# vislearn/HINT

Measured on AMD Instinct MI355X. Metric: train_samples_per_sec, higher is better.
Workload: dtype f32; 1 GPU; power_hint_8: d=6, 8 recursive coupling blocks, c_internal=[140, 70, 35, 17], batch 4096 per GPU; global_batch=4096, parallelism=dp1, hip_graph=True, steps_per_graph=1, input=batch resident in the captured step's input buffer (no per-step copy), rccl_world_size=1, backend=none (one process), gradient_allreduce=none (one process: clamp + Adam ride in the weight gradients' final reduction)

## Files before the change

hint_amd/csrc/hint_wl.hpp:

```cpp
#pragma once
#include "hint_rows.hpp"

namespace hint {

__device__ __forceinline__ f32x4 fma4(const f32x4 w, float s, const f32x4 a) {
    return f32x4{fmaf(w.x, s, a.x), fmaf(w.y, s, a.y), fmaf(w.z, s, a.z), fmaf(w.w, s, a.w)};
}
__device__ __forceinline__ float dot4(const f32x4 w, const f32x4 v, float a) {
    return fmaf(w.w, v.w, fmaf(w.z, v.z, fmaf(w.y, v.y, fmaf(w.x, v.x, a))));
}
__device__ __forceinline__ f32x4 relu4(const f32x4 v) { return f32x4{fmaxf(v.x, 0.f), fmaxf(v.y, 0.f), fmaxf(v.z, 0.f), fmaxf(v.w, 0.f)}; }
__device__ __forceinline__ f32x4 relu4m(const f32x4 v) {
    return f32x4{__builtin_amdgcn_fmed3f(v.x, 0.f, 3.0e38f), __builtin_amdgcn_fmed3f(v.y, 0.f, 3.0e38f),
                 __builtin_amdgcn_fmed3f(v.z, 0.f, 3.0e38f), __builtin_amdgcn_fmed3f(v.w, 0.f, 3.0e38f)};
}
__device__ __forceinline__ float kq_sum(float v) {
    const unsigned u = (unsigned)__float_as_int(v);
    const auto h = __builtin_amdgcn_permlane32_swap(u, u, false, false);
    const float a = __int_as_float((int)h[0]) + __int_as_float((int)h[1]);
    const unsigned ua = (unsigned)__float_as_int(a);
    const auto q = __builtin_amdgcn_permlane16_swap(ua, ua, false, false);
    return __int_as_float((int)q[0]) + __int_as_float((int)q[1]);
}

template <bool TRANS, typename WP>
__device__ __forceinline__ void wl_perm(float* dst, const float* src, int ld, WP w, int d, int lane) {
    const int m = lane & 15, kq = lane >> 4;
    float av[4], bv[4];
#pragma unroll
    for (int t = 0; t < 4; ++t) {
        const int k = 4 * t + kq;
        const int kc = k < d ? k : 0, mc = m < d ? m : 0;
        av[t] = TRANS ? w[mc * d + kc] : w[kc * d + mc];
        bv[t] = src[m * ld + kc];
    }
    f32x4 acc = zero4();
#pragma unroll
    for (int t = 0; t < 4; ++t) {
        if (4 * t < d) {
            const bool ok = 4 * t + kq < d;
            acc = mfma4((ok && m < d) ? av[t] : 0.f, ok ? bv[t] : 0.f, acc);
        }
    }
#pragma unroll
    for (int i = 0; i < 4; ++i)
        if (4 * kq + i < d) dst[m * ld + 4 * kq + i] = acc[i];
}

__device__ __forceinline__ void wl_store_share(float* __restrict__ dst, const float* tile, int ld, int d, float inv_d, int nvalid,
                                               int wave, int nw, int lane) {
    const int per = (ROWS * d + nw - 1) / nw;
    const int i = wave * per + lane;
    if (lane < per && i < nvalid) { const int r = fdiv(i, inv_d); dst[i] = tile[r * ld + (i - r * d)]; }
}

typedef unsigned wl_u32x4 __attribute__((ext_vector_type(4)));
__device__ __forceinline__ f32x4 wl_as_f32x4(wl_u32x4 v) { return __builtin_bit_cast(f32x4, v); }
__device__ __forceinline__ void wl_mask_by_bits(f32x4& v, int bits) {
    const float e[4] = {v.x, v.y, v.z, v.w};
    float o[4];
#pragma unroll
    for (int i = 0; i < 4; ++i) o[i] = __int_as_float(__float_as_int(e[i]) & __builtin_amdgcn_sbfe(bits, i, 1));
    v = f32x4{o[0], o[1], o[2], o[3]};
}

__device__ __forceinline__ f32x4 wl_layer1(const LDS_AS f32x4* q, const float (&vin)[4]) {
    const f32x4 qb = q[16], q0 = q[0], q1 = q[4], q2 = q[8], q3 = q[12];
    return fma4(q3, vin[3], fma4(q2, vin[2], fma4(q1, vin[1], fma4(q0, vin[0], qb))));
}

struct WlCtx {
    const GLOBAL_AS float* pk;
    const GLOBAL_AS float* pk_next;
    const GLOBAL_AS uint8_t* bits[2];
    const GLOBAL_AS uint8_t* bits_next[2];
    const LDS_AS int32_t* lrecs;
    const LDS_AS float* par;
    LDS_AS float* slab;
    const LDS_AS float* xs[2];
    const LDS_AS float* gst[2];
    LDS_AS float* scratch;
    GLOBAL_AS float* a2[2];
    GLOBAL_AS uint8_t* bits_out[2];
    GLOBAL_AS float* tw;
    int xld, gld, WT, slab_h;
    int sid, sid0;
    bool train, first_tile;
};

template <int KIND, int NR>
__device__ __forceinline__ void wl_load(f32x4 (&dst)[NEL], const GLOBAL_AS float* pk, const GLOBAL_AS uint8_t* const (&bits)[2],
                                        const RowU& r, int kb, const LaneOff& lo) {
    const __amdgpu_buffer_rsrc_t rw = __builtin_amdgcn_make_buffer_rsrc((void*)pk, 0, -1, 0x00020000);
#pragma unroll
    for (int j = 0; j < NTT; ++j) {
        const int jj = j < r.ntt ? j : r.ntt - 1;
        dst[j] = wl_as_f32x4(__builtin_amdgcn_raw_buffer_load_b128(rw, (int)lo.w, (r.base1 + jj * r.n1 + kb) * 1024, 0));
    }
// ... 194 lines not shown
    RecV nrec;
};
template <int KIND, int NR>
__device__ __forceinline__ void wl_rows(const WlCtx& c, f32x4 (&ring)[RING][NEL], WlCarry& cy, int r0, int r1, int rnext,
                                        bool other_block, int lane) {
    if (r0 >= r1) return;
    LaneOff lo;
    lo.w = (unsigned)lane * 16u; lo.b = (unsigned)(lane >> 4) * 16u; lo.l = (unsigned)lane;
    if (cy.held != r0) cy.nrec = wl_rec_fetch(c.lrecs, r0, lane);
    RowU cr = wl_rec_decode(cy.nrec);
    if (cy.primed != r0) wl_load<KIND, NR>(ring[0], c.pk, c.bits, cr, 0, lo);
    const int rlast = rnext >= 0 ? rnext : r1 - 1;
    cy.nrec = wl_rec_fetch(c.lrecs, r0 + 1 < r1 ? r0 + 1 : rlast, lane);
    f32x4 part[NR];
#pragma unroll
    for (int h = 0; h < NR; ++h) part[h] = zero4();
    for (int t = r0; t < r1; ++t) {
        const RowU nr = wl_rec_decode(cy.nrec);
        cy.nrec = wl_rec_fetch(c.lrecs, t + 2 < r1 ? t + 2 : rlast, lane);
        const bool hand = t + 1 == r1 && other_block;
#ifdef HINT_STAMPS
        const_cast<WlCtx&>(c).sid = 256 + ((c.sid0 >> 3) & 3) * 64 + (t - r0 < 2 ? t - r0 : 1) * 32;
#endif
        const GLOBAL_AS float* pkn = hand ? c.pk_next : c.pk;
        const GLOBAL_AS uint8_t* const bitsn[2] = {hand ? c.bits_next[0] : c.bits[0], hand ? c.bits_next[1] : c.bits[1]};
        wl_row<KIND, NR>(c, cr, nr, pkn, bitsn, ring, part, lo, lane);
        cr = nr;
    }
    cy.primed = rnext;
    cy.held = rlast;
}

template <int PR>
__device__ __forceinline__ void wl_par_issue(f32x4 (&pf)[PR], const GLOBAL_AS float* packed, const WlArgs& w, int tid, int nthreads) {
#pragma unroll
    for (int q = 0; q < PR; ++q) {
        int i = tid + q * nthreads;
        i = i < w.par_f4 ? i : w.par_f4 - 1;
        const int f = 4 * i;
        pf[q] = *(const GLOBAL_AS f32x4*)(packed + (f < w.par_bias ? f : f - w.par_bias + w.bias_src));
    }
}
__device__ __forceinline__ void wl_par_dma(const GLOBAL_AS float* packed, const WlArgs& w, const LDS_AS float* dst, int wave, int nw, int lane) {
    const int nchunk = (w.par_f4 + 63) >> 6;
    const unsigned base = (unsigned)(unsigned long long)dst;
    for (int c = wave; c < nchunk; c += nw) {
        int i = c * 64 + lane;
        i = i < w.par_f4 ? i : w.par_f4 - 1;
        const int f = 4 * i;
        const GLOBAL_AS float* src = packed + (f < w.par_bias ? f : f - w.par_bias + w.bias_src);
        const unsigned ldsb = (unsigned)rfl((int)(base + (unsigned)c * 1024u));
        unsigned keep;
        asm volatile("s_mov_b32 %0, m0\n\ts_mov_b32 m0, %2\n\ts_nop 0\n\tglobal_load_lds_dwordx4 %1, off\n\ts_mov_b32 m0, %0"
                     : "=&s"(keep) : "v"(src), "s"(ldsb) : "memory");
    }
}
__device__ __forceinline__ void wl_par_dma_wait() { asm volatile("s_waitcnt vmcnt(0)" ::: "memory"); }
template <int PR>
__device__ __forceinline__ void wl_par_commit(const f32x4 (&pf)[PR], float* dst, const WlArgs& w, int tid, int nthreads) {
#pragma unroll
    for (int q = 0; q < PR; ++q) {
        const int i = tid + q * nthreads;
        if (i < w.par_f4) ((f32x4*)dst)[i] = pf[q];
    }

}

}
```

hint_amd/csrc/hint_wl_bwd.hip:

```cpp
#include "hint_wl.hpp"

using namespace hint;

struct WlLevel { float x[WL_LV], s[WL_LV]; };
__device__ __forceinline__ void wl_level_issue(WlLevel& p, const float* __restrict__ xsrc, const float* __restrict__ ssrc,
                                               int d, int row0, int nvalid, int lane) {
    const size_t base = (size_t)row0 * d;
#pragma unroll
    for (int k = 0; k < WL_LV; ++k) {
        const int i = lane + 64 * k;
        const int ic = i < nvalid ? i : 0;
        p.x[k] = xsrc[base + ic];
        p.s[k] = ssrc[base + ic];
    }
}
__device__ __forceinline__ void wl_level_commit(const WlLevel& p, float* xs, float* sb, int ld, int d, int nvalid, int lane) {
    const float inv = frcp(d);
#pragma unroll
    for (int k = 0; k < WL_LV; ++k) {
        const int i = lane + 64 * k;
        if (i < ROWS * d) {
            const int r = fdiv(i, inv), j = i - r * d;
            xs[r * ld + j] = i < nvalid ? p.x[k] : 0.f;
            sb[r * ld + j] = i < nvalid ? p.s[k] : 0.f;
        }
    }
}

template <int NR, bool CH>
__global__ __launch_bounds__(64 * MAX_NW) __attribute__((amdgpu_waves_per_eu(2, 2))) void hint_wl_bwd_kernel(
    KArgs a, WlArgs w, ChainBlock one, const ChainBlock* __restrict__ chain, int n_chain,
    const float* __restrict__ x, const float* __restrict__ g_z, const float* __restrict__ g_J,
    float* __restrict__ g_x, float gz_scale, float gJ_const) {
    extern __shared__ __attribute__((aligned(16))) float lds[];
    const int tid = threadIdx.x, nthreads = blockDim.x;
    const int lane = tid & 63;
    const int wave = rfl(tid >> 6);
    const float inv_d = frcp(a.d);
    const Tables T = make_tables(a, lds);
    float* par = lds + w.off_par;
    float* slabs = lds + w.off_slab;
    float* ptab = lds + w.off_perm;
    float* gj = lds + w.off_misc;
    float* priv = lds + w.off_priv + wave * w.priv_stride;
    const int tl = ROWS * a.xld;
#define XSP(H) (priv + (H) * w.priv_tile)
#define SBP(H) (priv + (H) * w.priv_tile + tl)
#define G0P(H) (priv + (H) * w.priv_tile + 2 * tl)
#define GSTP(H) (priv + (H) * w.priv_tile + 4 * tl)
    float* scratch = priv + NR * w.priv_tile;
    const int par_floats = (4 * w.par_f4 + 255) & ~255;
    const int ntiles = (a.B + ROWS - 1) / ROWS;
    const int ngroups = (ntiles + NR - 1) / NR;
    const int pdd = a.d * a.d;
    const size_t lvl = (size_t)a.B * a.d;
    STAMP_DECL()
    copy_meta(a, lds, tid, nthreads);
    LDS_AS int32_t* lrecs = (LDS_AS int32_t*)(lds + w.off_recs);
    wl_stage_recs(lrecs, (const char*)a.recs + (size_t)a.total_rows * sizeof(RowRec), a.total_rows, tid, nthreads);
    if (a.perm_lds > 0) {
        for (int i = tid; i < n_chain * pdd; i += nthreads) {
            const int cbi = fdiv(i, frcp(pdd));
            const float* pp = CH ? chain[cbi].perm : one.perm;
            ptab[i] = pp != nullptr ? ((const GLOBAL_AS float*)pp)[i - cbi * pdd] : 0.f;
        }
    }
#define HINT_CB(I) chain_block<CH ? 1 : 2>(chain, one, I)
    int tr0 = 0, tr1 = 0, tgi = 0;
    bool tabs_ready = false;
#define LEVEL_SRC(TAPE, TOP, LV) ((LV) == 0 ? ((TOP) ? (TAPE) + (size_t)(a.n_levels - 1) * lvl : x) : (TAPE) + (size_t)((LV) - 1) * lvl)
#define BITS_A2(BLK, R0) ((const GLOBAL_AS uint8_t*)((BLK).actA1 + a.bits_off) + a.bits_stride + (size_t)((R0) >> 4) * (a.WT >> 4) * 64)

    for (int tg = blockIdx.x; tg < ngroups; tg += gridDim.x) {
        int row0[NR], nvalid[NR], rowt[NR];
#pragma unroll
        for (int h = 0; h < NR; ++h) {
            row0[h] = (tg * NR + h) * ROWS;
            const int rows = a.B - row0[h];
            nvalid[h] = (rows < 0 ? 0 : rows < ROWS ? rows : ROWS) * a.d;
            rowt[h] = row0[h] < ntiles * ROWS ? row0[h] : row0[0];
        }
        int gcur = 0;
#define GS(H) (G0P(H) + gcur)
#define GO(H) (G0P(H) + (tl - gcur))
#pragma unroll
        for (int h = 0; h < NR; ++h)
            for (int i = lane; i < ROWS * a.d; i += 64) {
                const int r = fdiv(i, inv_d);
                GS(h)[r * a.xld + (i - r * a.d)] = i < nvalid[h] ? g_z[(size_t)row0[h] * a.d + i] * gz_scale : 0.f;
            }
        if (tid < ROWS * NR) {
            const int h = tid >> 4, r = tid & 15;
            gj[tid] = ((tg * NR + h) * ROWS + r < a.B) ? (g_J != nullptr ? g_J[(tg * NR + h) * ROWS + r] : gJ_const) : 0.f;
        }
        {
            const GBlock lb = HINT_CB(n_chain - 1);
            const float* tape = (const float*)lb.tape;
            const bool top = lb.perm != nullptr || n_chain > 1;
            WlLevel lp[NR];
#pragma unroll
            for (int h = 0; h < NR; ++h)
                wl_level_issue(lp[h], LEVEL_SRC(tape, top, a.n_levels - 1), tape + (size_t)(2 * a.n_levels - 1) * lvl, a.d, rowt[h], nvalid[h], lane);
            f32x4 pf[NR == 2 ? WL_PAR_REGS2 : WL_PAR_REGS];
            wl_par_issue(pf, lb.packed, w, tid, nthreads);
#pragma unroll
            for (int h = 0; h < NR; ++h) wl_level_commit(lp[h], XSP(h), SBP(h), a.xld, a.d, nvalid[h], lane);
            wl_par_commit(pf, par, w, tid, nthreads);
        }
        __syncthreads();
        if (!tabs_ready) {
            const int b = lane <= a.n_groups ? lane : 0;
            const LDS_AS int32_t* gp = (const LDS_AS int32_t*)(T.groups + (b < a.n_groups ? b : 0));
            const int row_begin = gp[3], rngb = gp[6];
            tr0 = row_begin + T.rng[rngb + wave];
            tr1 = row_begin + T.rng[rngb + wave + 1];
            tgi = gp[7] | (T.rng[a.lop_cnt + b] << 8);
            tabs_ready = true;
        }
        int phase = 0;
        WlCarry primed; primed.primed = -1; primed.held = -1;
        f32x4 ring[RING][NEL];

        for (int cb = n_chain - 1; cb >= 0; --cb) {
            const int wi = n_chain - 1 - cb;
            const bool has_next = cb > 0;
            const GBlock blk = HINT_CB(cb);
            const GBlock nblk = HINT_CB(has_next ? cb - 1 : cb);
            const float* perm = (const float*)blk.perm;
            const float* tape = (const float*)blk.tape;
            const bool top = perm != nullptr || cb > 0;
            float* wsGST = (float*)blk.wsGST;
            const int tsel = wi & (a.nw - 1);
            constexpr bool PAR_DMA = NR == 2;
            f32x4 pf[PAR_DMA ? 1 : WL_PAR_REGS];
            if constexpr (PAR_DMA) { if (has_next) wl_par_dma(nblk.packed, w, (const LDS_AS float*)(par + ((wi + 1) & 1) * par_floats), wave, a.nw, lane); }
            else wl_par_issue(pf, nblk.packed, w, tid, nthreads);

            WlCtx c;
            c.pk = blk.packed; c.pk_next = nblk.packed;
#pragma unroll
            for (int h = 0; h < 2; ++h) {
                const int hh = h < NR ? h : 0;
                c.bits[h] = BITS_A2(blk, rowt[hh]); c.bits_next[h] = BITS_A2(nblk, rowt[hh]);
                c.xs[h] = (const LDS_AS float*)XSP(hh); c.gst[h] = (const LDS_AS float*)GSTP(hh);
                c.a2[h] = nullptr; c.bits_out[h] = nullptr;
            }
            c.lrecs = lrecs;
            c.par = (const LDS_AS float*)(par + (wi & 1) * par_floats);
            c.scratch = (LDS_AS float*)scratch;
            c.tw = blk.wsSlab + a.thin_slab_off + (size_t)blockIdx.x * a.tw_floats;
            c.xld = a.xld; c.gld = a.gld; c.WT = a.WT; c.slab_h = w.slab_floats; c.train = true; c.first_tile = tg == (int)blockIdx.x;

            for (int gi = a.n_groups; gi >= 0; --gi) {
                const int slot = gi > 0 ? gi - 1 : a.n_groups;
                const bool tail_only = gi == 0;
                const int ginfo = wl_lane_get(tgi, slot);
                struct { int level; } g;
                g.level = ginfo & 0xff;
                const int lop0 = slot * a.d;
                const float* slab_prev = slabs + ((phase + 1) & 1) * NR * w.slab_floats;
                const int sid = (wi * (a.n_groups + 1) + (a.n_groups - gi)) * 8;
                (void)sid;
                STAMP(sid + 0)
                const int nact = ginfo >> 8;
                for (int idx = lane; idx < ROWS * nact; idx += 64) {
                    const int row = idx & 15, kk = idx >> 4;
// ... 24 lines not shown
#pragma unroll
                                for (int u = 0; u < 4; ++u) gb[h] += u < sl_n ? v[u] : 0.f;
                                if (more) for (int sl = 4; sl < sl_n; ++sl) gb[h] += sp[sl * 64];
                            }
                        }
#pragma unroll
                        for (int h = 0; h < NR; ++h) {
                            if (colb == col) gval[h] = gb[h];
                            else GS(h)[row * a.xld + colb] = gb[h];
                        }
                    }
                    if (!tail_only && cp_ls >= 0) {
#pragma unroll
                        for (int h = 0; h < NR; ++h) {
                            const float s = SBP(h)[row * a.xld + col];
                            const float aa = a.alpha * atanf(s);
                            const float ea = expf(aa);
                            const float l = XSP(h)[row * a.xld + col];
                            const float ga = gval[h] * ea * l + gj[h * ROWS + row];
                            const float gsv = ga * a.alpha * __builtin_amdgcn_rcpf(1.f + s * s);
                            GSTP(h)[row * a.gld + cp_ls] = gsv;
                            GSTP(h)[row * a.gld + cp_lt] = gval[h];
                            if (wave == tsel && row0[h] < ntiles * ROWS) {
                                float* go = wsGST + (size_t)(row0[h] + row) * a.ST;
                                go[cp_gs] = gsv;
                                go[cp_gt] = gval[h];
                            }
                            gval[h] *= ea;
                        }
                    }
#pragma unroll
                    for (int h = 0; h < NR; ++h) GS(h)[row * a.xld + col] = gval[h];
                }
                c.sid0 = sid; c.sid = 256;
                STAMP(sid + 1)
                if (tail_only) break;

                WlLevel lp[NR];
                bool lp_pending = false;
                {
                    const bool block_switch = slot == 0;
                    int nlevel = a.n_levels - 1;
                    if (!block_switch) nlevel = wl_lane_get(tgi, slot - 1) & 0xff;
                    if (block_switch ? cb > 0 : nlevel != g.level) {
                        const float* ntape = block_switch ? (const float*)nblk.tape : tape;
                        const bool ntop = block_switch ? (nblk.perm != nullptr || cb > 1) : top;
#pragma unroll
                        for (int h = 0; h < NR; ++h)
                            wl_level_issue(lp[h], LEVEL_SRC(ntape, ntop, nlevel), ntape + (size_t)(a.n_levels + nlevel) * lvl, a.d, rowt[h], nvalid[h], lane);
                        lp_pending = true;
                    }
                }
                c.slab = (LDS_AS float*)(slabs + (phase & 1) * NR * w.slab_floats);
                ++phase;
                {
                    int rnext = -1;
                    const bool wrap = slot == 0;
                    if (!wrap || has_next) {
                        const int gn = wrap ? a.n_groups - 1 : slot - 1;
                        const int n0 = wl_lane_get(tr0, gn), n1 = wl_lane_get(tr1, gn);
                        if (n0 < n1) rnext = n0;
                    }
                    if (wave >= 4) __builtin_amdgcn_s_setprio(1);
                    wl_rows<K_BWD, NR>(c, ring, primed, wl_lane_get(tr0, slot), wl_lane_get(tr1, slot), rnext, wrap, lane);
                    __builtin_amdgcn_s_setprio(0);
                }
                STAMP(sid + 2)
                if (gi == a.n_groups) {
                    if constexpr (PAR_DMA) wl_par_dma_wait();
                    else wl_par_commit(pf, par + ((wi + 1) & 1) * par_floats, w, tid, nthreads);
                }
                if (lp_pending) {
#pragma unroll
                    for (int h = 0; h < NR; ++h) wl_level_commit(lp[h], XSP(h), SBP(h), a.xld, a.d, nvalid[h], lane);
                }
                STAMP(sid + 3)
                lds_barrier();
                STAMP(sid + 4)
            }
            if (blk.g_add != nullptr) {
#pragma unroll
                for (int h = 0; h < NR; ++h)
                    for (int i = lane; i < nvalid[h]; i += 64) {
                        const int r = fdiv(i, inv_d);
                        GS(h)[r * a.xld + (i - r * a.d)] += blk.g_add[(size_t)row0[h] * a.d + i];
                    }
            }
            if (perm != nullptr) {
#pragma unroll
                for (int h = 0; h < NR; ++h) {
                    if (a.perm_lds > 0) wl_perm<true>(GO(h), GS(h), a.xld, (const LDS_AS float*)(ptab + cb * pdd), a.d, lane);
                    else wl_perm<true>(GO(h), GS(h), a.xld, (const GLOBAL_AS float*)perm, a.d, lane);
                }
                gcur = tl - gcur;
            }
        }
        if (wave == 0) {
#pragma unroll
            for (int h = 0; h < NR; ++h)
                for (int i = lane; i < nvalid[h]; i += 64) { const int r = fdiv(i, inv_d); g_x[(size_t)row0[h] * a.d + i] = GS(h)[r * a.xld + (i - r * a.d)]; }
        }
        __syncthreads();
#undef GS
#undef GO
    }
    STAMP_FLUSH(a.stamps)
#undef HINT_CB
#undef LEVEL_SRC
#undef BITS_A2
#undef XSP
#undef SBP
#undef G0P
#undef GSTP
}

namespace hint {

hipError_t launch_wl_bwd(const KArgs& a, const WlArgs& w, int lds_bytes, int grid, const ChainBlock& one,
                         const ChainBlock* chain, int n_chain, const float* x, const float* g_z, const float* g_J,
                         float* g_x, float gz_scale, float gJ_const, hipStream_t stream) {
#define HINT_LAUNCH(NRV, CHV)                                                                                        \
    hipLaunchKernelGGL((hint_wl_bwd_kernel<NRV, CHV>), dim3(grid), dim3(64 * a.nw), lds_bytes, stream, a, w, one, chain, n_chain, x, \
                       g_z, g_J, g_x, gz_scale, gJ_const)
// ... 18 lines not shown
```

hint_amd/csrc/hint_wl_fwd.hip:

```cpp
#include "hint_wl.hpp"

using namespace hint;

template <bool REV, int NR, bool CH>
__global__ __launch_bounds__(64 * MAX_NW) __attribute__((amdgpu_waves_per_eu(2, 2))) void hint_wl_apply_kernel(
    KArgs a, WlArgs w, ChainBlock one, const ChainBlock* __restrict__ chain, int n_chain,
    const float* __restrict__ x, float* __restrict__ z, float* __restrict__ J, const float* __restrict__ J_in,
    float* __restrict__ loss_acc, float noise, const unsigned long long* __restrict__ rng_state,
    float* __restrict__ x_noisy) {
    extern __shared__ __attribute__((aligned(16))) float lds[];
    const int tid = threadIdx.x, nthreads = blockDim.x;
    const int lane = tid & 63, m = lane & 15, kq = lane >> 4;
    const int wave = rfl(tid >> 6);
    const float inv_d = frcp(a.d);
    const Tables T = make_tables(a, lds);
    float* par = lds + w.off_par;
    float* slabs = lds + w.off_slab;
    float* ptab = lds + w.off_perm;
    float* priv = lds + w.off_priv + wave * w.priv_stride;
    const int par_floats = (4 * w.par_f4 + 255) & ~255;
    const int ntiles = (a.B + ROWS - 1) / ROWS;
    const int ngroups = (ntiles + NR - 1) / NR;
    const int pdd = a.d * a.d;
    const size_t lvl = (size_t)a.B * a.d;
    STAMP_DECL()
    copy_meta(a, lds, tid, nthreads);
    LDS_AS int32_t* lrecs = (LDS_AS int32_t*)(lds + w.off_recs);
    wl_stage_recs(lrecs, a.recs, a.total_rows, tid, nthreads);
    if (a.perm_lds > 0) {
        for (int i = tid; i < n_chain * pdd; i += nthreads) {
            const int cbi = fdiv(i, frcp(pdd));
            const float* pp = CH ? chain[cbi].perm : one.perm;
            ptab[i] = pp != nullptr ? ((const GLOBAL_AS float*)pp)[i - cbi * pdd] : 0.f;
        }
    }
#define HINT_CB(I) chain_block<CH ? 1 : 2>(chain, one, I)
    int tr0 = 0, tr1 = 0, tgi = 0;
    bool tabs_ready = false;

    for (int tg = blockIdx.x; tg < ngroups; tg += gridDim.x) {
        int row0[NR], nvalid[NR];
#pragma unroll
        for (int h = 0; h < NR; ++h) {
            row0[h] = (tg * NR + h) * ROWS;
            const int rows = a.B - row0[h];
            nvalid[h] = (rows < 0 ? 0 : rows < ROWS ? rows : ROWS) * a.d;
        }
        int xcur = 0;
        const int xflip = ROWS * a.xld;
#define XS(H) (priv + (H) * w.priv_tile + xcur)
#define XO(H) (priv + (H) * w.priv_tile + (xflip - xcur))
#pragma unroll
        for (int h = 0; h < NR; ++h)
            for (int i = lane; i < ROWS * a.d; i += 64) {
                const int r = fdiv(i, inv_d);
                XS(h)[r * a.xld + (i - r * a.d)] = i < nvalid[h] ? x[(size_t)row0[h] * a.d + i] : 0.f;
            }
        if (!REV && rng_state != nullptr) {
            const unsigned long long seed = rng_state[0], step = rng_state[1];
#pragma unroll
            for (int h = 0; h < NR; ++h) {
                for (int q = lane; 4 * q < nvalid[h]; q += 64) {
                    float nz[4];
                    philox_normal4(seed, step, (unsigned)(((size_t)row0[h] * a.d) / 4 + (size_t)q), nz);
#pragma unroll
                    for (int e = 0; e < 4; ++e) {
                        const int i = 4 * q + e;
                        if (i < nvalid[h]) { const int r = fdiv(i, inv_d); XS(h)[r * a.xld + (i - r * a.d)] += noise * nz[e]; }
                    }
                }
                if (x_noisy != nullptr && wave == 0)
                    for (int i = lane; i < nvalid[h]; i += 64) { const int r = fdiv(i, inv_d); x_noisy[(size_t)row0[h] * a.d + i] = XS(h)[r * a.xld + (i - r * a.d)]; }
            }
        }
        {
            const GBlock b0 = HINT_CB(REV ? n_chain - 1 : 0);
            f32x4 pf[NR == 2 ? WL_PAR_REGS2 : WL_PAR_REGS];
            wl_par_issue(pf, b0.packed, w, tid, nthreads);
            wl_par_commit(pf, par, w, tid, nthreads);
        }
        __syncthreads();
        if (!tabs_ready) {
            const int e = lane < a.n_groups ? lane : 0;
            const LDS_AS int32_t* gp = (const LDS_AS int32_t*)(T.groups + (REV ? a.n_groups - 1 - e : e));
            const int row_begin = gp[3], rngb = gp[6];
            tr0 = row_begin + T.rng[rngb + wave];
            tr1 = row_begin + T.rng[rngb + wave + 1];
            tgi = gp[4] | (gp[5] << 16) | (gp[7] << 24) | (gp[8] << 30);
            tabs_ready = true;
        }
        float jpart[NR];
#pragma unroll
        for (int h = 0; h < NR; ++h) jpart[h] = 0.f;
        int phase = 0;
        WlCarry primed; primed.primed = -1; primed.held = -1;
        f32x4 ring[RING][NEL];

        for (int cb = 0; cb < n_chain; ++cb) {
            const int bi = REV ? n_chain - 1 - cb : cb;
            const bool has_next = cb + 1 < n_chain;
            const GBlock blk = HINT_CB(bi);
            const GBlock nblk = HINT_CB(has_next ? (REV ? bi - 1 : bi + 1) : bi);
            const float* perm = (const float*)blk.perm;
            float* tape = (float*)blk.tape;
            const bool train = !REV && blk.actA1 != nullptr;
            const int tsel = cb & (a.nw - 1);
            if (!REV && perm != nullptr) {
#pragma unroll
                for (int h = 0; h < NR; ++h) {
                    if (a.perm_lds > 0) wl_perm<false>(XO(h), XS(h), a.xld, (const LDS_AS float*)(ptab + bi * pdd), a.d, lane);
                    else wl_perm<false>(XO(h), XS(h), a.xld, (const GLOBAL_AS float*)perm, a.d, lane);
                }
                xcur = xflip - xcur;
            }
            if (!REV && tape != nullptr && (perm != nullptr || cb > 0)) {
#pragma unroll
                for (int h = 0; h < NR; ++h)
                    wl_store_share(tape + (size_t)(a.n_levels - 1) * lvl + (size_t)row0[h] * a.d, XS(h), a.xld, a.d, inv_d, nvalid[h], wave, a.nw, lane);
            }
            f32x4 pf[NR == 2 ? WL_PAR_REGS2 : WL_PAR_REGS];
            wl_par_issue(pf, nblk.packed, w, tid, nthreads);

            WlCtx c;
            c.pk = blk.packed; c.pk_next = nblk.packed;
            c.lrecs = lrecs;
            c.par = (const LDS_AS float*)(par + (cb & 1) * par_floats);
            c.scratch = nullptr; c.tw = nullptr;
#pragma unroll
            for (int h = 0; h < 2; ++h) {
                const int hh = h < NR ? h : 0;
                c.bits[h] = nullptr; c.bits_next[h] = nullptr; c.gst[h] = nullptr;
                const bool tile_ok = train && h < NR && row0[hh] < ntiles * ROWS;
                c.a2[h] = tile_ok ? blk.actA1 + a.a2_off + (size_t)row0[hh] * a.WT : nullptr;
                c.bits_out[h] = tile_ok ? (GLOBAL_AS uint8_t*)(blk.actA1 + a.bits_off) + a.bits_stride + (size_t)(row0[hh] >> 4) * (a.WT >> 4) * 64 : nullptr;
            }
            c.xld = a.xld; c.gld = 0; c.WT = a.WT; c.slab_h = w.slab_floats; c.train = train; c.first_tile = false;

            for (int gi = 0; gi < a.n_groups; ++gi) {
                const int ginfo = wl_lane_get(tgi, gi);
                struct { int ent_begin, ent_cnt, level, level_last; } g;
                g.ent_begin = ginfo & 0xffff; g.ent_cnt = (ginfo >> 16) & 0xff; g.level = (ginfo >> 24) & 0x3f; g.level_last = (ginfo >> 30) & 1;
                float* slab = slabs + (phase & 1) * NR * w.slab_floats;
                ++phase;
#pragma unroll
                for (int h = 0; h < 2; ++h) c.xs[h] = (const LDS_AS float*)XS(h < NR ? h : 0);
                c.slab = (LDS_AS float*)slab;
                const int sid = (cb * a.n_groups + gi) * 8;
                (void)sid;
                c.sid0 = sid; c.sid = 256;
                STAMP(sid + 0)
                {
                    int rnext = -1;
                    const bool wrap = gi + 1 == a.n_groups;
                    if (!wrap || has_next) {
                        const int en = wrap ? 0 : gi + 1;
                        const int n0 = wl_lane_get(tr0, en), n1 = wl_lane_get(tr1, en);
                        if (n0 < n1) rnext = n0;
// ... 27 lines not shown
#pragma unroll
                        for (int u = 0; u < 4; ++u) { s += u < sl_ns ? vs[u] : 0.f; t += u < sl_nt ? vt[u] : 0.f; }
                        if (more) {
                            for (int sl = 4; sl < sl_ns; ++sl) s += sp[sl * 64];
                            for (int sl = 4; sl < sl_nt; ++sl) t += tp[sl * 64];
                        }
                        const float aa = a.alpha * atanf(s);
                        if (act && train && tape != nullptr && wave == tsel && row0[h] + m < a.B)
                            tape[(size_t)(a.n_levels + g.level) * lvl + (size_t)(row0[h] + m) * a.d + xcol] = s;
                        float xn;
                        if (!REV) { xn = expf(aa) * xold[h] + t; jpart[h] += act ? aa : 0.f; }
                        else      { xn = (xold[h] - t) * __builtin_amdgcn_rcpf(expf(aa)); jpart[h] -= act ? aa : 0.f; }
                        if (act) XS(h)[m * a.xld + xcol] = xn;
                    }
                    if (ps + 1 < npass) {
                        const int en = 4 * (ps + 1) + kq;
                        ent = *(const LDS_AS i32x4*)(T.ents + g.ent_begin + (en < g.ent_cnt ? en : 0));
#pragma unroll
                        for (int h = 0; h < NR; ++h) xold[h] = XS(h)[m * a.xld + (ent.x & 0xffff)];
                    }
                }
                STAMP(sid + 4)
                if (gi == 0) {
                    wl_par_commit(pf, par + ((cb + 1) & 1) * par_floats, w, tid, nthreads);
                    if (a.n_groups == 1) lds_barrier();
                }
                if (!REV && tape != nullptr && g.level_last && g.level < a.n_levels - 1) {
#pragma unroll
                    for (int h = 0; h < NR; ++h)
                        wl_store_share(tape + (size_t)g.level * lvl + (size_t)row0[h] * a.d, XS(h), a.xld, a.d, inv_d, nvalid[h], wave, a.nw, lane);
                }
                STAMP(sid + 5)
            }
            if (REV && perm != nullptr) {
#pragma unroll
                for (int h = 0; h < NR; ++h) {
                    if (a.perm_lds > 0) wl_perm<true>(XO(h), XS(h), a.xld, (const LDS_AS float*)(ptab + bi * pdd), a.d, lane);
                    else wl_perm<true>(XO(h), XS(h), a.xld, (const GLOBAL_AS float*)perm, a.d, lane);
                }
                xcur = xflip - xcur;
            }
        }
        float zz = 0.f, js = 0.f;
#pragma unroll
        for (int h = 0; h < NR; ++h) {
            const bool rok = row0[h] + m < a.B;
            const float jrow = kq_sum(jpart[h]) + ((J_in != nullptr && rok) ? J_in[row0[h] + m] : 0.f);
            if (wave == 0) {
                for (int i = lane; i < nvalid[h]; i += 64) {
                    const int r = fdiv(i, inv_d);
                    const float v = XS(h)[r * a.xld + (i - r * a.d)];
                    z[(size_t)row0[h] * a.d + i] = v;
                    zz += v * v;
                }
                if (kq == 0 && rok) { J[row0[h] + m] = jrow; js += jrow; }
            }
        }
        if (wave == 0 && loss_acc != nullptr) {
            for (int o = 32; o > 0; o >>= 1) { zz += __shfl_xor(zz, o, 64); js += __shfl_xor(js, o, 64); }
            if (lane == 0) {
                float* slot = loss_acc + 2 * (blockIdx.x & 63);
                atomicAdd(slot, 0.5f * zz);
                atomicAdd(slot + 1, js);
            }
        }
        __syncthreads();
#undef XS
#undef XO
    }
    STAMP_FLUSH(a.stamps)
#undef HINT_CB
}

namespace hint {

hipError_t launch_wl_apply(bool rev, const KArgs& a, const WlArgs& w, int lds_bytes, int grid, const ChainBlock& one,
                           const ChainBlock* chain, int n_chain, const float* x, float* z, float* J, const float* J_in,
                           float* loss_acc, float noise, const unsigned long long* rng_state, float* x_noisy,
// ... 29 lines not shown
```

Before: 14.46 million samples/s.

## Pin kernel args in SGPRs, load next-block pointers lazily, rematerialize lane ids

Copies the kernel arguments into locals and pins them in scalar registers through inline-asm moves. The next chain block's pointers are now read from the constant-address-space chain array only when they are needed, and the per-tile bit-offset deltas are precomputed. Lane and thread indices are passed as separately rematerialized values so the compiler does not keep extra VGPRs live across the long loops. The goal is to cut register pressure and spills in the fused forward and backward kernels, at the cost of asm barriers that can constrain the scheduler.

After: 14.62 million samples/s, median of 6. 1.01x the previous value.

```diff
diff --git a/hint_amd/csrc/hint_wl.hpp b/hint_amd/csrc/hint_wl.hpp
--- a/hint_amd/csrc/hint_wl.hpp
+++ b/hint_amd/csrc/hint_wl.hpp
@@ -23,9 +23,29 @@
     return __int_as_float((int)q[0]) + __int_as_float((int)q[1]);
 }
 
+#if defined(__HIP_DEVICE_COMPILE__)
+#define WL_DEV_ASM(...) __VA_ARGS__
+#else
+#define WL_DEV_ASM(...)
+#endif
+template <typename T>
+__device__ __forceinline__ void wl_own(T& v) {
+    static_assert(sizeof(T) == 4 || sizeof(T) == 8, "one register or a pair");
+    T o = v;
+    if constexpr (sizeof(T) == 4) { WL_DEV_ASM(asm volatile("s_mov_b32 %0, %1" : "=s"(o) : "s"(v))); }
+    else { WL_DEV_ASM(asm volatile("s_mov_b64 %0, %1" : "=s"(o) : "s"(v))); }
+    v = o;
+}
+template <typename T>
+__device__ __forceinline__ T wl_here(T v) { WL_DEV_ASM(asm volatile("" : "+s"(v))); return v; }
+
+__device__ __forceinline__ int wl_fresh(int& lane_o) { WL_DEV_ASM(asm volatile("" : "+v"(lane_o))); return lane_o; }
+
 template <bool TRANS, typename WP>
-__device__ __forceinline__ void wl_perm(float* dst, const float* src, int ld, WP w, int d, int lane) {
+__device__ __forceinline__ void wl_perm(float* dst, const float* src, int ld, WP w, int d, int lane, int lane_f) {
     const int m = lane & 15, kq = lane >> 4;
+    const int mf = lane_f & 15, kqf = lane_f >> 4;
+    const int df = wl_here(d);
     float av[4], bv[4];
 #pragma unroll
     for (int t = 0; t < 4; ++t) {
@@ -37,21 +57,21 @@
     f32x4 acc = zero4();
 #pragma unroll
     for (int t = 0; t < 4; ++t) {
-        if (4 * t < d) {
-            const bool ok = 4 * t + kq < d;
-            acc = mfma4((ok && m < d) ? av[t] : 0.f, ok ? bv[t] : 0.f, acc);
+        if (4 * t < df) {
+            const bool ok = kqf + 4 * t < df;
+            acc = mfma4((ok && mf < df) ? av[t] : 0.f, ok ? bv[t] : 0.f, acc);
         }
     }
 #pragma unroll
     for (int i = 0; i < 4; ++i)
-        if (4 * kq + i < d) dst[m * ld + 4 * kq + i] = acc[i];
-}
-
-__device__ __forceinline__ void wl_store_share(float* __restrict__ dst, const float* tile, int ld, int d, float inv_d, int nvalid,
-                                               int wave, int nw, int lane) {
+        if (4 * kqf + i < df) dst[m * ld + 4 * kq + i] = acc[i];
+}
+
+__device__ __forceinline__ void wl_store_share(GLOBAL_AS float* __restrict__ dst, const float* tile, int ld, int d, float inv_d, int nvalid,
+                                               int wave, int nw, int lane, int lane_f) {
     const int per = (ROWS * d + nw - 1) / nw;
     const int i = wave * per + lane;
-    if (lane < per && i < nvalid) { const int r = fdiv(i, inv_d); dst[i] = tile[r * ld + (i - r * d)]; }
+    if (lane_f < per && lane_f < nvalid - wave * per) { const int r = fdiv(i, inv_d); dst[i] = tile[r * ld + (i - r * d)]; }
 }
 
 typedef unsigned wl_u32x4 __attribute__((ext_vector_type(4)));
@@ -69,11 +89,33 @@
     return fma4(q3, vin[3], fma4(q2, vin[2], fma4(q1, vin[1], fma4(q0, vin[0], qb))));
 }
 
+typedef const __attribute__((address_space(4))) ChainBlock* WlChain;
+struct WlBlk {
+    const GLOBAL_AS float* packed;
+    const GLOBAL_AS float* perm;
+    GLOBAL_AS float* tape;
+    GLOBAL_AS float* actA1;
+    GLOBAL_AS float* wsGST;
+    GLOBAL_AS float* wsSlab;
+    const GLOBAL_AS float* g_add;
+};
+#define WL_BLK_FIELD(F) ((GLOBAL_AS float*)(CH ? chain[i].F : one.F))
+template <bool CH>
+__device__ __forceinline__ WlBlk wl_block(WlChain chain, const ChainBlock& one, int i) {
+    WlBlk b;
+    b.packed = WL_BLK_FIELD(packed); b.perm = WL_BLK_FIELD(perm); b.tape = WL_BLK_FIELD(tape); b.actA1 = WL_BLK_FIELD(actA1);
+    b.wsGST = WL_BLK_FIELD(wsGST); b.wsSlab = WL_BLK_FIELD(wsSlab); b.g_add = WL_BLK_FIELD(g_add);
+    WL_DEV_ASM(asm("" : "+s"(b.packed)); asm("" : "+s"(b.perm)); asm("" : "+s"(b.tape)); asm("" : "+s"(b.actA1));
+               asm("" : "+s"(b.wsGST)); asm("" : "+s"(b.wsSlab)); asm("" : "+s"(b.g_add)));
+    return b;
+}
+#undef WL_BLK_FIELD
+
 struct WlCtx {
     const GLOBAL_AS float* pk;
-    const GLOBAL_AS float* pk_next;
+    WlChain next;
     const GLOBAL_AS uint8_t* bits[2];
-    const GLOBAL_AS uint8_t* bits_next[2];
+    long long bits_delta[2];
     const LDS_AS int32_t* lrecs;
     const LDS_AS float* par;
     LDS_AS float* slab;
@@ -314,8 +356,17 @@
 #ifdef HINT_STAMPS
         const_cast<WlCtx&>(c).sid = 256 + ((c.sid0 >> 3) & 3) * 64 + (t - r0 < 2 ? t - r0 : 1) * 32;
 #endif
-        const GLOBAL_AS float* pkn = hand ? c.pk_next : c.pk;
-        const GLOBAL_AS uint8_t* const bitsn[2] = {hand ? c.bits_next[0] : c.bits[0], hand ? c.bits_next[1] : c.bits[1]};
+        const GLOBAL_AS float* pkn = c.pk;
+        const GLOBAL_AS uint8_t* bitsn[2] = {c.bits[0], c.bits[1]};
+        if (hand && c.next != nullptr) {
+            const WlChain nx = wl_here(c.next);
+            pkn = (const GLOBAL_AS float*)nx->packed;
+            if (KIND == K_BWD) {
+                const GLOBAL_AS uint8_t* an = (const GLOBAL_AS uint8_t*)nx->actA1;
+#pragma unroll
+                for (int h = 0; h < 2; ++h) bitsn[h] = an + c.bits_delta[h < NR ? h : 0];
+            }
+        }
         wl_row<KIND, NR>(c, cr, nr, pkn, bitsn, ring, part, lo, lane);
         cr = nr;
     }
@@ -349,13 +400,13 @@
 }
 __device__ __forceinline__ void wl_par_dma_wait() { asm volatile("s_waitcnt vmcnt(0)" ::: "memory"); }
 template <int PR>
-__device__ __forceinline__ void wl_par_commit(const f32x4 (&pf)[PR], float* dst, const WlArgs& w, int tid, int nthreads) {
+__device__ __forceinline__ void wl_par_commit(const f32x4 (&pf)[PR], float* dst, const WlArgs& w, int tid, int tid_f, int nthreads) {
 #pragma unroll
     for (int q = 0; q < PR; ++q) {
         const int i = tid + q * nthreads;
-        if (i < w.par_f4) ((f32x4*)dst)[i] = pf[q];
-    }
-
-}
-
-}
+        if (tid_f + q * nthreads < w.par_f4) ((f32x4*)dst)[i] = pf[q];
+    }
+
+}
+
+}
diff --git a/hint_amd/csrc/hint_wl_bwd.hip b/hint_amd/csrc/hint_wl_bwd.hip
--- a/hint_amd/csrc/hint_wl_bwd.hip
+++ b/hint_amd/csrc/hint_wl_bwd.hip
@@ -3,7 +3,7 @@
 using namespace hint;
 
 struct WlLevel { float x[WL_LV], s[WL_LV]; };
-__device__ __forceinline__ void wl_level_issue(WlLevel& p, const float* __restrict__ xsrc, const float* __restrict__ ssrc,
+__device__ __forceinline__ void wl_level_issue(WlLevel& p, const GLOBAL_AS float* __restrict__ xsrc, const GLOBAL_AS float* __restrict__ ssrc,
                                                int d, int row0, int nvalid, int lane) {
     const size_t base = (size_t)row0 * d;
 #pragma unroll
@@ -14,28 +14,42 @@
         p.s[k] = ssrc[base + ic];
     }
 }
-__device__ __forceinline__ void wl_level_commit(const WlLevel& p, float* xs, float* sb, int ld, int d, int nvalid, int lane) {
+__device__ __forceinline__ void wl_level_commit(const WlLevel& p, float* xs, float* sb, int ld, int d, int nvalid, int lane, int lane_f) {
     const float inv = frcp(d);
 #pragma unroll
     for (int k = 0; k < WL_LV; ++k) {
         const int i = lane + 64 * k;
-        if (i < ROWS * d) {
+        const int i_f = lane_f + 64 * k;
+        if (i_f < ROWS * d) {
             const int r = fdiv(i, inv), j = i - r * d;
-            xs[r * ld + j] = i < nvalid ? p.x[k] : 0.f;
-            sb[r * ld + j] = i < nvalid ? p.s[k] : 0.f;
+            const bool ok = i_f < nvalid;
+            xs[r * ld + j] = ok ? p.x[k] : 0.f;
+            sb[r * ld + j] = ok ? p.s[k] : 0.f;
         }
     }
 }
 
 template <int NR, bool CH>
 __global__ __launch_bounds__(64 * MAX_NW) __attribute__((amdgpu_waves_per_eu(2, 2))) void hint_wl_bwd_kernel(
-    KArgs a, WlArgs w, ChainBlock one, const ChainBlock* __restrict__ chain, int n_chain,
+    KArgs a_, WlArgs w_, ChainBlock one, const ChainBlock* __restrict__ chain, int n_chain,
     const float* __restrict__ x, const float* __restrict__ g_z, const float* __restrict__ g_J,
     float* __restrict__ g_x, float gz_scale, float gJ_const) {
     extern __shared__ __attribute__((aligned(16))) float lds[];
+    KArgs a = a_;
+    WlArgs w = w_;
+    wl_own(a.d); wl_own(a.xld); wl_own(a.gld); wl_own(a.B); wl_own(a.n_levels); wl_own(a.n_groups); wl_own(a.nw); wl_own(a.alpha);
+    wl_own(a.ST); wl_own(a.WT); wl_own(a.bits_off); wl_own(a.bits_stride); wl_own(a.thin_slab_off); wl_own(a.tw_floats); wl_own(a.perm_lds);
+    WlChain chc = (WlChain)(unsigned long long)chain;
+    const GLOBAL_AS float* xg = (const GLOBAL_AS float*)x;
+    const GLOBAL_AS float* gzg = (const GLOBAL_AS float*)g_z;
+    const GLOBAL_AS float* gJg = (const GLOBAL_AS float*)g_J;
+    GLOBAL_AS float* gxg = (GLOBAL_AS float*)g_x;
+    wl_own(chc); wl_own(n_chain); wl_own(xg); wl_own(gzg); wl_own(gJg); wl_own(gxg); wl_own(gz_scale); wl_own(gJ_const);
+    wl_own(w.slab_floats); wl_own(w.priv_tile); wl_own(w.par_f4); wl_own(w.par_bias); wl_own(w.bias_src);
     const int tid = threadIdx.x, nthreads = blockDim.x;
     const int lane = tid & 63;
     const int wave = rfl(tid >> 6);
+    int lane_o = lane, tid_o = tid;
     const float inv_d = frcp(a.d);
     const Tables T = make_tables(a, lds);
     float* par = lds + w.off_par;
@@ -65,11 +79,10 @@
             ptab[i] = pp != nullptr ? ((const GLOBAL_AS float*)pp)[i - cbi * pdd] : 0.f;
         }
     }
-#define HINT_CB(I) chain_block<CH ? 1 : 2>(chain, one, I)
+#define HINT_CB(I) wl_block<CH>(chc, one, I)
     int tr0 = 0, tr1 = 0, tgi = 0;
     bool tabs_ready = false;
-#define LEVEL_SRC(TAPE, TOP, LV) ((LV) == 0 ? ((TOP) ? (TAPE) + (size_t)(a.n_levels - 1) * lvl : x) : (TAPE) + (size_t)((LV) - 1) * lvl)
-#define BITS_A2(BLK, R0) ((const GLOBAL_AS uint8_t*)((BLK).actA1 + a.bits_off) + a.bits_stride + (size_t)((R0) >> 4) * (a.WT >> 4) * 64)
+#define LEVEL_SRC(TAPE, TOP, LV) ((LV) == 0 ? ((TOP) ? (TAPE) + (size_t)(a.n_levels - 1) * lvl : xg) : (TAPE) + (size_t)((LV) - 1) * lvl)
 
     for (int tg = blockIdx.x; tg < ngroups; tg += gridDim.x) {
         int row0[NR], nvalid[NR], rowt[NR];
@@ -80,6 +93,12 @@
             nvalid[h] = (rows < 0 ? 0 : rows < ROWS ? rows : ROWS) * a.d;
             rowt[h] = row0[h] < ntiles * ROWS ? row0[h] : row0[0];
         }
+        long long bits_delta[NR];
+#pragma unroll
+        for (int h = 0; h < NR; ++h) {
+            bits_delta[h] = (long long)a.bits_off * 4 + a.bits_stride + (long long)(rowt[h] >> 4) * (a.WT >> 4) * 64;
+            wl_own(bits_delta[h]);
+        }
         int gcur = 0;
 #define GS(H) (G0P(H) + gcur)
 #define GO(H) (G0P(H) + (tl - gcur))
@@ -87,15 +106,15 @@
         for (int h = 0; h < NR; ++h)
             for (int i = lane; i < ROWS * a.d; i += 64) {
                 const int r = fdiv(i, inv_d);
-                GS(h)[r * a.xld + (i - r * a.d)] = i < nvalid[h] ? g_z[(size_t)row0[h] * a.d + i] * gz_scale : 0.f;
+                GS(h)[r * a.xld + (i - r * a.d)] = i < nvalid[h] ? gzg[(size_t)row0[h] * a.d + i] * gz_scale : 0.f;
             }
         if (tid < ROWS * NR) {
             const int h = tid >> 4, r = tid & 15;
-            gj[tid] = ((tg * NR + h) * ROWS + r < a.B) ? (g_J != nullptr ? g_J[(tg * NR + h) * ROWS + r] : gJ_const) : 0.f;
+            gj[tid] = ((tg * NR + h) * ROWS + r < a.B) ? (gJg != nullptr ? gJg[(tg * NR + h) * ROWS + r] : gJ_const) : 0.f;
         }
         {
-            const GBlock lb = HINT_CB(n_chain - 1);
-            const float* tape = (const float*)lb.tape;
+            const WlBlk lb = HINT_CB(n_chain - 1);
+            const GLOBAL_AS float* tape = lb.tape;
             const bool top = lb.perm != nullptr || n_chain > 1;
             WlLevel lp[NR];
 #pragma unroll
@@ -104,8 +123,8 @@
             f32x4 pf[NR == 2 ? WL_PAR_REGS2 : WL_PAR_REGS];
             wl_par_issue(pf, lb.packed, w, tid, nthreads);
 #pragma unroll
-            for (int h = 0; h < NR; ++h) wl_level_commit(lp[h], XSP(h), SBP(h), a.xld, a.d, nvalid[h], lane);
-            wl_par_commit(pf, par, w, tid, nthreads);
+            for (int h = 0; h < NR; ++h) wl_level_commit(lp[h], XSP(h), SBP(h), a.xld, a.d, nvalid[h], lane, lane);
+            wl_par_commit(pf, par, w, tid, tid, nthreads);
         }
         __syncthreads();
         if (!tabs_ready) {
@@ -124,24 +143,25 @@
         for (int cb = n_chain - 1; cb >= 0; --cb) {
             const int wi = n_chain - 1 - cb;
             const bool has_next = cb > 0;
-            const GBlock blk = HINT_CB(cb);
-            const GBlock nblk = HINT_CB(has_next ? cb - 1 : cb);
-            const float* perm = (const float*)blk.perm;
-            const float* tape = (const float*)blk.tape;
+            const WlBlk blk = HINT_CB(cb);
+            const int nbi = has_next ? cb - 1 : cb;
+            const GLOBAL_AS float* perm = blk.perm;
+            const GLOBAL_AS float* tape = blk.tape;
             const bool top = perm != nullptr || cb > 0;
-            float* wsGST = (float*)blk.wsGST;
+            GLOBAL_AS float* wsGST = blk.wsGST;
             const int tsel = wi & (a.nw - 1);
             constexpr bool PAR_DMA = NR == 2;
             f32x4 pf[PAR_DMA ? 1 : WL_PAR_REGS];
-            if constexpr (PAR_DMA) { if (has_next) wl_par_dma(nblk.packed, w, (const LDS_AS float*)(par + ((wi + 1) & 1) * par_floats), wave, a.nw, lane); }
-            else wl_par_issue(pf, nblk.packed, w, tid, nthreads);
+            if constexpr (PAR_DMA) { if (has_next) wl_par_dma(HINT_CB(nbi).packed, w, (const LDS_AS float*)(par + ((wi + 1) & 1) * par_floats), wave, a.nw, lane); }
+            else wl_par_issue(pf, HINT_CB(nbi).packed, w, tid, nthreads);
 
             WlCtx c;
-            c.pk = blk.packed; c.pk_next = nblk.packed;
+            c.pk = blk.packed; c.next = CH && has_next ? chc + nbi : nullptr;
 #pragma unroll
             for (int h = 0; h < 2; ++h) {
                 const int hh = h < NR ? h : 0;
-                c.bits[h] = BITS_A2(blk, rowt[hh]); c.bits_next[h] = BITS_A2(nblk, rowt[hh]);
+                c.bits_delta[h] = bits_delta[hh];
+                c.bits[h] = (const GLOBAL_AS uint8_t*)blk.actA1 + bits_delta[hh];
                 c.xs[h] = (const LDS_AS float*)XSP(hh); c.gst[h] = (const LDS_AS float*)GSTP(hh);
                 c.a2[h] = nullptr; c.bits_out[h] = nullptr;
             }
@@ -212,7 +232,7 @@
                             GSTP(h)[row * a.gld + cp_ls] = gsv;
                             GSTP(h)[row * a.gld + cp_lt] = gval[h];
                             if (wave == tsel && row0[h] < ntiles * ROWS) {
-                                float* go = wsGST + (size_t)(row0[h] + row) * a.ST;
+                                GLOBAL_AS float* go = wsGST + (size_t)(row0[h] + row) * a.ST;
                                 go[cp_gs] = gsv;
                                 go[cp_gt] = gval[h];
                             }
@@ -233,8 +253,9 @@
                     int nlevel = a.n_levels - 1;
                     if (!block_switch) nlevel = wl_lane_get(tgi, slot - 1) & 0xff;
                     if (block_switch ? cb > 0 : nlevel != g.level) {
-                        const float* ntape = block_switch ? (const float*)nblk.tape : tape;
-                        const bool ntop = block_switch ? (nblk.perm != nullptr || cb > 1) : top;
+                        const GLOBAL_AS float* ntape = tape;
+                        bool ntop = top;
+                        if (block_switch) { const WlBlk nblk = HINT_CB(wl_here(nbi)); ntape = nblk.tape; ntop = nblk.perm != nullptr || cb > 1; }
 #pragma unroll
                         for (int h = 0; h < NR; ++h)
                             wl_level_issue(lp[h], LEVEL_SRC(ntape, ntop, nlevel), ntape + (size_t)(a.n_levels + nlevel) * lvl, a.d, rowt[h], nvalid[h], lane);
@@ -258,11 +279,11 @@
                 STAMP(sid + 2)
                 if (gi == a.n_groups) {
                     if constexpr (PAR_DMA) wl_par_dma_wait();
-                    else wl_par_commit(pf, par + ((wi + 1) & 1) * par_floats, w, tid, nthreads);
+                    else wl_par_commit(pf, par + ((wi + 1) & 1) * par_floats, w, tid, wl_fresh(tid_o), nthreads);
                 }
                 if (lp_pending) {
 #pragma unroll
-                    for (int h = 0; h < NR; ++h) wl_level_commit(lp[h], XSP(h), SBP(h), a.xld, a.d, nvalid[h], lane);
+                    for (int h = 0; h < NR; ++h) wl_level_commit(lp[h], XSP(h), SBP(h), a.xld, a.d, nvalid[h], lane, wl_fresh(lane_o));
                 }
                 STAMP(sid + 3)
                 lds_barrier();
@@ -279,8 +300,8 @@
             if (perm != nullptr) {
 #pragma unroll
                 for (int h = 0; h < NR; ++h) {
-                    if (a.perm_lds > 0) wl_perm<true>(GO(h), GS(h), a.xld, (const LDS_AS float*)(ptab + cb * pdd), a.d, lane);
-                    else wl_perm<true>(GO(h), GS(h), a.xld, (const GLOBAL_AS float*)perm, a.d, lane);
+                    if (a.perm_lds > 0) wl_perm<true>(GO(h), GS(h), a.xld, (const LDS_AS float*)(ptab + cb * pdd), a.d, lane, wl_fresh(lane_o));
+                    else wl_perm<true>(GO(h), GS(h), a.xld, (const GLOBAL_AS float*)perm, a.d, lane, wl_fresh(lane_o));
                 }
                 gcur = tl - gcur;
             }
@@ -288,7 +309,7 @@
         if (wave == 0) {
 #pragma unroll
             for (int h = 0; h < NR; ++h)
-                for (int i = lane; i < nvalid[h]; i += 64) { const int r = fdiv(i, inv_d); g_x[(size_t)row0[h] * a.d + i] = GS(h)[r * a.xld + (i - r * a.d)]; }
+                for (int i = lane; i < nvalid[h]; i += 64) { const int r = fdiv(i, inv_d); gxg[(size_t)row0[h] * a.d + i] = GS(h)[r * a.xld + (i - r * a.d)]; }
         }
         __syncthreads();
 #undef GS
diff --git a/hint_amd/csrc/hint_wl_fwd.hip b/hint_amd/csrc/hint_wl_fwd.hip
--- a/hint_amd/csrc/hint_wl_fwd.hip
+++ b/hint_amd/csrc/hint_wl_fwd.hip
@@ -4,14 +4,25 @@
 
 template <bool REV, int NR, bool CH>
 __global__ __launch_bounds__(64 * MAX_NW) __attribute__((amdgpu_waves_per_eu(2, 2))) void hint_wl_apply_kernel(
-    KArgs a, WlArgs w, ChainBlock one, const ChainBlock* __restrict__ chain, int n_chain,
+    KArgs a_, WlArgs w_, ChainBlock one, const ChainBlock* __restrict__ chain, int n_chain,
     const float* __restrict__ x, float* __restrict__ z, float* __restrict__ J, const float* __restrict__ J_in,
     float* __restrict__ loss_acc, float noise, const unsigned long long* __restrict__ rng_state,
     float* __restrict__ x_noisy) {
     extern __shared__ __attribute__((aligned(16))) float lds[];
+    KArgs a = a_;
+    WlArgs w = w_;
+    wl_own(a.d); wl_own(a.xld); wl_own(a.B); wl_own(a.n_levels); wl_own(a.n_groups); wl_own(a.nw); wl_own(a.alpha);
+    wl_own(a.WT); wl_own(a.a2_off); wl_own(a.bits_off); wl_own(a.bits_stride); wl_own(a.perm_lds);
+    WlChain chc = (WlChain)(unsigned long long)chain;
+    GLOBAL_AS float* zg = (GLOBAL_AS float*)z;
+    GLOBAL_AS float* Jg = (GLOBAL_AS float*)J;
+    const GLOBAL_AS float* Jing = (const GLOBAL_AS float*)J_in;
+    wl_own(chc); wl_own(n_chain); wl_own(zg); wl_own(Jg); wl_own(Jing);
+    wl_own(w.slab_floats); wl_own(w.priv_tile); wl_own(w.par_f4); wl_own(w.par_bias); wl_own(w.bias_src);
     const int tid = threadIdx.x, nthreads = blockDim.x;
     const int lane = tid & 63, m = lane & 15, kq = lane >> 4;
     const int wave = rfl(tid >> 6);
+    int lane_o = lane, tid_o = tid;
     const float inv_d = frcp(a.d);
     const Tables T = make_tables(a, lds);
     float* par = lds + w.off_par;
@@ -34,7 +45,7 @@
             ptab[i] = pp != nullptr ? ((const GLOBAL_AS float*)pp)[i - cbi * pdd] : 0.f;
         }
     }
-#define HINT_CB(I) chain_block<CH ? 1 : 2>(chain, one, I)
+#define HINT_CB(I) wl_block<CH>(chc, one, I)
     int tr0 = 0, tr1 = 0, tgi = 0;
     bool tabs_ready = false;
 
@@ -46,6 +57,13 @@
             const int rows = a.B - row0[h];
             nvalid[h] = (rows < 0 ? 0 : rows < ROWS ? rows : ROWS) * a.d;
         }
+        long long a2_delta[NR], bo_delta[NR];
+#pragma unroll
+        for (int h = 0; h < NR; ++h) {
+            a2_delta[h] = (long long)a.a2_off + (long long)row0[h] * a.WT;
+            bo_delta[h] = (long long)a.bits_off * 4 + a.bits_stride + (long long)(row0[h] >> 4) * (a.WT >> 4) * 64;
+            wl_own(a2_delta[h]); wl_own(bo_delta[h]);
+        }
         int xcur = 0;
         const int xflip = ROWS * a.xld;
 #define XS(H) (priv + (H) * w.priv_tile + xcur)
@@ -74,10 +92,10 @@
             }
         }
         {
-            const GBlock b0 = HINT_CB(REV ? n_chain - 1 : 0);
+            const WlBlk b0 = HINT_CB(REV ? n_chain - 1 : 0);
             f32x4 pf[NR == 2 ? WL_PAR_REGS2 : WL_PAR_REGS];
             wl_par_issue(pf, b0.packed, w, tid, nthreads);
-            wl_par_commit(pf, par, w, tid, nthreads);
+            wl_par_commit(pf, par, w, tid, tid, nthreads);
         }
         __syncthreads();
         if (!tabs_ready) {
@@ -99,40 +117,40 @@
         for (int cb = 0; cb < n_chain; ++cb) {
             const int bi = REV ? n_chain - 1 - cb : cb;
             const bool has_next = cb + 1 < n_chain;
-            const GBlock blk = HINT_CB(bi);
-            const GBlock nblk = HINT_CB(has_next ? (REV ? bi - 1 : bi + 1) : bi);
-            const float* perm = (const float*)blk.perm;
-            float* tape = (float*)blk.tape;
+            const WlBlk blk = HINT_CB(bi);
+            const int nbi = has_next ? (REV ? bi - 1 : bi + 1) : bi;
+            const GLOBAL_AS float* perm = blk.perm;
+            GLOBAL_AS float* tape = blk.tape;
             const bool train = !REV && blk.actA1 != nullptr;
             const int tsel = cb & (a.nw - 1);
             if (!REV && perm != nullptr) {
 #pragma unroll
                 for (int h = 0; h < NR; ++h) {
-                    if (a.perm_lds > 0) wl_perm<false>(XO(h), XS(h), a.xld, (const LDS_AS float*)(ptab + bi * pdd), a.d, lane);
-                    else wl_perm<false>(XO(h), XS(h), a.xld, (const GLOBAL_AS float*)perm, a.d, lane);
+                    if (a.perm_lds > 0) wl_perm<false>(XO(h), XS(h), a.xld, (const LDS_AS float*)(ptab + bi * pdd), a.d, lane, wl_fresh(lane_o));
+                    else wl_perm<false>(XO(h), XS(h), a.xld, (const GLOBAL_AS float*)perm, a.d, lane, wl_fresh(lane_o));
                 }
                 xcur = xflip - xcur;
             }
             if (!REV && tape != nullptr && (perm != nullptr || cb > 0)) {
 #pragma unroll
                 for (int h = 0; h < NR; ++h)
-                    wl_store_share(tape + (size_t)(a.n_levels - 1) * lvl + (size_t)row0[h] * a.d, XS(h), a.xld, a.d, inv_d, nvalid[h], wave, a.nw, lane);
+                    wl_store_share(tape + (size_t)(a.n_levels - 1) * lvl + (size_t)row0[h] * a.d, XS(h), a.xld, a.d, inv_d, nvalid[h], wave, a.nw, lane, wl_fresh(lane_o));
             }
             f32x4 pf[NR == 2 ? WL_PAR_REGS2 : WL_PAR_REGS];
-            wl_par_issue(pf, nblk.packed, w, tid, nthreads);
+            wl_par_issue(pf, HINT_CB(nbi).packed, w, tid, nthreads);
 
             WlCtx c;
-            c.pk = blk.packed; c.pk_next = nblk.packed;
+            c.pk = blk.packed; c.next = CH && has_next ? chc + nbi : nullptr;
             c.lrecs = lrecs;
             c.par = (const LDS_AS float*)(par + (cb & 1) * par_floats);
             c.scratch = nullptr; c.tw = nullptr;
 #pragma unroll
             for (int h = 0; h < 2; ++h) {
                 const int hh = h < NR ? h : 0;
-                c.bits[h] = nullptr; c.bits_next[h] = nullptr; c.gst[h] = nullptr;
+                c.bits[h] = nullptr; c.bits_delta[h] = 0; c.gst[h] = nullptr;
                 const bool tile_ok = train && h < NR && row0[hh] < ntiles * ROWS;
-                c.a2[h] = tile_ok ? blk.actA1 + a.a2_off + (size_t)row0[hh] * a.WT : nullptr;
-                c.bits_out[h] = tile_ok ? (GLOBAL_AS uint8_t*)(blk.actA1 + a.bits_off) + a.bits_stride + (size_t)(row0[hh] >> 4) * (a.WT >> 4) * 64 : nullptr;
+                c.a2[h] = tile_ok ? blk.actA1 + a2_delta[hh] : nullptr;
+                c.bits_out[h] = tile_ok ? (GLOBAL_AS uint8_t*)blk.actA1 + bo_delta[hh] : nullptr;
             }
             c.xld = a.xld; c.gld = 0; c.WT = a.WT; c.slab_h = w.slab_floats; c.train = train; c.first_tile = false;
 
@@ -206,21 +224,21 @@
                 }
                 STAMP(sid + 4)
                 if (gi == 0) {
-                    wl_par_commit(pf, par + ((cb + 1) & 1) * par_floats, w, tid, nthreads);
+                    wl_par_commit(pf, par + ((cb + 1) & 1) * par_floats, w, tid, wl_fresh(tid_o), nthreads);
                     if (a.n_groups == 1) lds_barrier();
                 }
                 if (!REV && tape != nullptr && g.level_last && g.level < a.n_levels - 1) {
 #pragma unroll
                     for (int h = 0; h < NR; ++h)
-                        wl_store_share(tape + (size_t)g.level * lvl + (size_t)row0[h] * a.d, XS(h), a.xld, a.d, inv_d, nvalid[h], wave, a.nw, lane);
+                        wl_store_share(tape + (size_t)g.level * lvl + (size_t)row0[h] * a.d, XS(h), a.xld, a.d, inv_d, nvalid[h], wave, a.nw, lane, wl_fresh(lane_o));
                 }
                 STAMP(sid + 5)
             }
             if (REV && perm != nullptr) {
 #pragma unroll
                 for (int h = 0; h < NR; ++h) {
-                    if (a.perm_lds > 0) wl_perm<true>(XO(h), XS(h), a.xld, (const LDS_AS float*)(ptab + bi * pdd), a.d, lane);
-                    else wl_perm<true>(XO(h), XS(h), a.xld, (const GLOBAL_AS float*)perm, a.d, lane);
+                    if (a.perm_lds > 0) wl_perm<true>(XO(h), XS(h), a.xld, (const LDS_AS float*)(ptab + bi * pdd), a.d, lane, wl_fresh(lane_o));
+                    else wl_perm<true>(XO(h), XS(h), a.xld, (const GLOBAL_AS float*)perm, a.d, lane, wl_fresh(lane_o));
                 }
                 xcur = xflip - xcur;
             }
@@ -229,15 +247,15 @@
 #pragma unroll
         for (int h = 0; h < NR; ++h) {
             const bool rok = row0[h] + m < a.B;
-            const float jrow = kq_sum(jpart[h]) + ((J_in != nullptr && rok) ? J_in[row0[h] + m] : 0.f);
+            const float jrow = kq_sum(jpart[h]) + ((Jing != nullptr && rok) ? Jing[row0[h] + m] : 0.f);
             if (wave == 0) {
                 for (int i = lane; i < nvalid[h]; i += 64) {
                     const int r = fdiv(i, inv_d);
                     const float v = XS(h)[r * a.xld + (i - r * a.d)];
-                    z[(size_t)row0[h] * a.d + i] = v;
+                    zg[(size_t)row0[h] * a.d + i] = v;
                     zz += v * v;
                 }
-                if (kq == 0 && rok) { J[row0[h] + m] = jrow; js += jrow; }
+                if (kq == 0 && rok) { Jg[row0[h] + m] = jrow; js += jrow; }
             }
         }
         if (wave == 0 && loss_acc != nullptr) {
```
